# lilinitsy/skele-raytracer

Hardware: AMD Instinct MI355X
Metric: Mrays/sec + frame ms, 1920x1080 gillum=16 spheres2.scn (higher is better)
Workload: dtype f32

## Files before the change

### skele_raytracer_amd/csrc/scene_host.cpp

```cpp
#include "scene_host.h"

#include <cstdarg>
#include <cstdio>
#include <cstdlib>
#include <cstring>
#include <algorithm>
#include <cmath>
#include <fstream>

static thread_local char g_err[512] = "";

void skr_set_error(const char *fmt, ...)
{
	va_list ap;
	va_start(ap, fmt);
	vsnprintf(g_err, sizeof g_err, fmt, ap);
	va_end(ap);
}

extern "C" const char *skr_last_error(void) { return g_err; }

namespace {

int read_floats(const char *p, float *dst, int n)
// ... 218 lines not shown
	const float reach2 = std::nextafter((float) (reach * reach), INFINITY);
	const double D = std::sqrt((double) reach2) * (1.0 + 0x1p-16);
	const double eta = 0x1p-16;
	std::vector<double> cell_dir, cell_theta;
	cube_cells(SKR_SHADOW_CELLS, cell_dir, cell_theta);
	for(double &t : cell_theta) t = t * (1.0 + 0x1p-20) + 0x1p-16;
	std::vector<uint32_t> masks((size_t) nl * SKR_SHADOW_TABLE_WORDS, 0u);
	for(int l = 0; l < nl; l++)
	{
		double lp[3];
		light_pos(l, lp);
		const double lmax = std::max(std::fabs(lp[0]), std::max(std::fabs(lp[1]), std::fabs(lp[2])));
		const double eps_o = 2.0 * std::sqrt(3.0) * (1e-6 + 0x1p-23 * (lmax + D + 1e-6));
		for(int k = 0; k < ns; k++)
		{
			const double q[3] = {sph_geom[k].x - lp[0], sph_geom[k].y - lp[1], sph_geom[k].z - lp[2]};
			const double r2 = sph_geom[k].w, qq = q[0] * q[0] + q[1] * q[1] + q[2] * q[2], qn = std::sqrt(qq);
			const double E = (qn + D + eps_o) * (1.0 + 0x1p-20);
			const double rk = std::sqrt(r2 + 0x1p-16 * (E * E + r2)) + 0x1p-20 * E;
			const double S = qn + rk;
			const double base = rk + eps_o + eta * (S + D + eps_o) / (1.0 - eta) + 0x1p-30 * qn;
			for(int c = 0; c < SKR_SHADOW_TABLE_WORDS; c++)
			{
				const double *wc = &cell_dir[3 * (size_t) c];
				const double s = q[0] * wc[0] + q[1] * wc[1] + q[2] * wc[2];
				const double dist = std::sqrt(std::max(0.0, qq - s * s));
				if(dist <= base + cell_theta[c] * S) masks[(size_t) l * SKR_SHADOW_TABLE_WORDS + c] |= 1u << k;
			}
		}
	}
	shadow_masks.swap(masks);
	shadow_reach2 = reach2;
}

struct BallSphere {
	double v[3], dist;
	double rk;
	double behind, reach;
	bool meets;
};
static BallSphere ball_sphere(const double *q, double rho, const double *C, double r2)
{
	BallSphere b;
	for(int c = 0; c < 3; c++) b.v[c] = C[c] - q[c];
	b.dist = std::sqrt(b.v[0] * b.v[0] + b.v[1] * b.v[1] + b.v[2] * b.v[2]);
	const double E = (b.dist + rho) * (1.0 + 0x1p-20);
	b.rk = std::sqrt(r2 + 0x1p-16 * (E * E + r2)) + 0x1p-20 * E;
	const double tol = 0x1p-30 * (b.dist + rho + b.rk);
	b.behind = rho + 0x1p-16 * E + tol;
	b.reach = b.rk + rho + tol;
	b.meets = b.dist <= b.reach;
	return b;
}
struct ConeSphere {
	double cos_lo, min_sin;
};
static ConeSphere cone_sphere(const double *v, double dist, const double *w, double ct, double st)
{
	const double cp = (v[0] * w[0] + v[1] * w[1] + v[2] * w[2]) / dist;
	const double x = v[1] * w[2] - v[2] * w[1], y = v[2] * w[0] - v[0] * w[2], z = v[0] * w[1] - v[1] * w[0];
	const double sp = std::sqrt(x * x + y * y + z * z) / dist;
	const bool lo0 = cp >= ct;
	const bool hipi = cp <= -ct;
	const double sin_lo = lo0 ? 0.0 : sp * ct - cp * st;
	const double sin_hi = hipi ? 0.0 : sp * ct + cp * st;
	return ConeSphere{lo0 ? 1.0 : cp * ct + sp * st, std::max(0.0, std::min(sin_lo, sin_hi))};
}
static bool cone_ahead(const ConeSphere &c, double dist, double behind) { return dist * c.cos_lo + behind >= 0.0; }
static bool cone_line_touches(const ConeSphere &c, double dist, double reach) { return dist * c.min_sin <= reach; }
static bool ball_cone_touches(const BallSphere &b, const double *w, double ct, double st)
{
	if(b.meets) return true;
	const ConeSphere c = cone_sphere(b.v, b.dist, w, ct, st);
	return cone_ahead(c, b.dist, b.behind) && cone_line_touches(c, b.dist, b.reach);
}
static void gi_ball_bits(const double *q, double rho, const double *C, double r2, uint32_t bit, const std::vector<double> &cell_dir,
						 const std::vector<double> &cth, const std::vector<double> &sth, uint32_t *row)
{
	const BallSphere b = ball_sphere(q, rho, C, r2);
	for(int e = 0; e < SKR_GI_ROW_ENTRIES; e++)
		if(ball_cone_touches(b, &cell_dir[3 * (size_t) e], cth[e], sth[e])) row[e] |= bit;
}

void skr_scene::build_gi_masks()
{
	gi_table.clear();
	gi_grid[0] = gi_grid[1] = SkrGiGrid{};
	gi_mask_word = 0;
	gi_wide = 0;
	const int ns = info.n_spheres;
	if(ns < 1 || ns > SKR_GI_MAX_SPHERES || info.n_triangles > 0) return;
	std::vector<double> C((size_t) 3 * ns), r2(ns), rad(ns);
	for(int k = 0; k < ns; k++)
	{
		C[3 * k] = sph_geom[k].x;
		C[3 * k + 1] = sph_geom[k].y;
		C[3 * k + 2] = sph_geom[k].z;
		r2[k] = sph_geom[k].w;
		rad[k] = std::sqrt(r2[k]);
		for(int c = 0; c < 3; c++)
			if(!(std::fabs(C[3 * k + c]) < 1e6)) return;
		if(!(rad[k] < 1e6)) return;
	}
	std::vector<double> sorted(rad);
	std::sort(sorted.begin(), sorted.end());
	const double small = 4.0 * sorted[ns / 2];
	double flo[3] = {INFINITY, INFINITY, INFINITY}, fhi[3] = {-INFINITY, -INFINITY, -INFINITY}, alo[3] = {INFINITY, INFINITY, INFINITY},
		   ahi[3] = {-INFINITY, -INFINITY, -INFINITY}, rsmall = 0.0;
	for(int k = 0; k < ns; k++)
		for(int c = 0; c < 3; c++)
		{
			alo[c] = std::min(alo[c], C[3 * k + c] - rad[k]);
			ahi[c] = std::max(ahi[c], C[3 * k + c] + rad[k]);
			if(rad[k] <= small)
			{
				flo[c] = std::min(flo[c], C[3 * k + c] - rad[k]);
				fhi[c] = std::max(fhi[c], C[3 * k + c] + rad[k]);
				rsmall = std::max(rsmall, rad[k]);
			}
		}
	double ext_f = 0.0;
	for(int c = 0; c < 3; c++)
	{
		flo[c] -= 2.0 * rsmall;
		fhi[c] += 2.0 * rsmall;
		ext_f = std::max(ext_f, fhi[c] - flo[c]);
	}
	if(!(ext_f > 1e-6)) return;
	double clo[3], chi[3], ext_c = 0.0;
	for(int c = 0; c < 3; c++)
	{
		clo[c] = std::min(flo[c], std::max(alo[c], flo[c] - ext_f));
		chi[c] = std::max(fhi[c], std::min(ahi[c], fhi[c] + ext_f));
		ext_c = std::max(ext_c, chi[c] - clo[c]);
	}
	gi_wide = ns > 16 ? 1 : 0;
	const size_t row_bytes = (size_t) SKR_GI_ROW_ENTRIES * (gi_wide ? 4 : 2);
	struct Cell {
		double q[3], rho;
	};
	std::vector<Cell> cells;
	std::vector<int32_t> index;
	double hh[2] = {0.0, 0.0};
	bool fits = false;
	for(int attempt = 0; attempt < 64 && !fits; attempt++)
	{
		const double grow = std::pow(1.15, attempt);
		cells.clear();
		index.clear();
		for(int g = 0; g < 2; g++)
		{
			SkrGiGrid &G = gi_grid[g];
			const double *lo = g ? clo : flo, *hi = g ? chi : fhi;
			G.inv = (float) (1.0 / ((g ? ext_c / 16.0 : ext_f / 32.0) * grow));
			hh[g] = 1.0 / (double) G.inv;
			for(int c = 0; c < 3; c++)
			{
				float l = (float) lo[c];
				if((double) l > lo[c]) l = std::nextafter(l, -INFINITY);
				G.lo[c] = l;
				G.n[c] = std::max(1, std::min(256, (int) std::ceil((hi[c] - (double) l) / hh[g])));
				G.n_f[c] = (float) G.n[c];
			}
			G.base = (int32_t) index.size();
			const int n0 = G.n[0], n1 = G.n[1], n2 = G.n[2];
			const double pad = 0x1p-18 * std::max(n0, std::max(n1, n2)) * hh[g];
			const double rho = std::sqrt(3.0) * (0.5 * hh[g] + pad) * (1.0 + 0x1p-20);
			for(int k = 0; k < n2; k++)
				for(int j = 0; j < n1; j++)
					for(int i = 0; i < n0; i++)
					{
						const int ijk[3] = {i, j, k};
						Cell cl;
						bool inside_fine = g == 1;
						for(int c = 0; c < 3; c++)
						{
							cl.q[c] = (double) G.lo[c] + (ijk[c] + 0.5) * hh[g];
							const double f0 = (double) gi_grid[0].lo[c], f1 = f0 + gi_grid[0].n[c] * hh[0];
							inside_fine = inside_fine && cl.q[c] - 0.5 * hh[g] >= f0 && cl.q[c] + 0.5 * hh[g] <= f1;
						}
						cl.rho = rho;
						bool near = false;
						for(int s = 0; s < ns && !near && !inside_fine; s++)
						{
							const double dx = C[3 * s] - cl.q[0], dy = C[3 * s + 1] - cl.q[1], dz = C[3 * s + 2] - cl.q[2];
							const double dist = std::sqrt(dx * dx + dy * dy + dz * dz);
							near = std::fabs(dist - rad[s]) <= rho + 1e-4 + 0x1p-16 * (dist + rad[s]);
						}
						index.push_back(near ? (int32_t) cells.size() : -1);
						if(near) cells.push_back(cl);
					}
		}
		fits = ((index.size() + 1) & ~(size_t) 1) * 4 + cells.size() * row_bytes <= SKR_GI_MAX_BYTES;
	}
	if(!fits || cells.empty()) return;
	std::vector<double> cell_dir, cell_theta;
	cube_cells(SKR_GI_DIR_CELLS, cell_dir, cell_theta);
	std::vector<double> cth(SKR_GI_ROW_ENTRIES), sth(SKR_GI_ROW_ENTRIES);
	for(int e = 0; e < SKR_GI_ROW_ENTRIES; e++)
	{
		const double t = cell_theta[e] * (1.0 + 0x1p-20) + 0x1p-40;
		cth[e] = std::cos(t);
		sth[e] = std::sin(t);
	}
	std::vector<uint32_t> masks(cells.size() * SKR_GI_ROW_ENTRIES, 0u);
	for(size_t ci = 0; ci < cells.size(); ci++)
		for(int k = 0; k < ns; k++) gi_ball_bits(cells[ci].q, cells[ci].rho, &C[3 * k], r2[k], 1u << k, cell_dir, cth, sth, &masks[ci * SKR_GI_ROW_ENTRIES]);
	const size_t n_index = (index.size() + 1) & ~(size_t) 1;
	const size_t n_mask_words = gi_wide ? masks.size() : masks.size() / 2;
	std::vector<uint32_t> table((n_index + n_mask_words + 3) & ~(size_t) 3, 0u);
	memcpy(table.data(), index.data(), index.size() * 4);
	if(gi_wide) memcpy(&table[n_index], masks.data(), masks.size() * 4);
	else
		for(size_t e = 0; e < masks.size(); e += 2) table[n_index + e / 2] = masks[e] | masks[e + 1] << 16;
	gi_mask_word = (uint32_t) n_index;
	gi_table.swap(table);
}

struct SurfaceShell {
	float tau;
	double R_lo, R_hi;
};
static SurfaceShell surface_shell(double r2)
{
	SurfaceShell sh;
	sh.tau = std::sqrt(r2) > 1e-3 ? (float) (r2 * 0x1p-7) : -1.0f;
	sh.R_lo = std::sqrt(std::max(0.0, (r2 - sh.tau) * (1.0 - 0x1p-20))) * (1.0 - 0x1p-22);
	sh.R_hi = std::sqrt((r2 + std::max(0.0f, sh.tau)) * (1.0 + 0x1p-20)) * (1.0 + 0x1p-22);
	return sh;
}
static void surface_patch_ball(const double *C, double rad, const SurfaceShell &sh, const double *w, double th, double *q, double &rho)
{
	const double h = rad * std::cos(th);
	for(int c = 0; c < 3; c++) q[c] = C[c] + h * w[c];
	double far = 0.0;
	for(double R : {sh.R_lo, sh.R_hi}) far = std::max(far, std::sqrt(std::max(0.0, R * R + h * h - 2.0 * R * h * std::cos(th))));
	double cmax = 0.0;
	for(int c = 0; c < 3; c++) cmax = std::max(cmax, std::fabs(C[c]));
	rho = far * (1.0 + 0x1p-20) + 0x1p-30 * (cmax + rad);
}
static void surface_cells(int g, std::vector<double> &dir, std::vector<double> &theta)
{
	dir.clear();
	theta.clear();
	if(g) cube_cells(g, dir, theta);
	for(double &t : theta) t = t * (1.0 + 0x1p-20) + 0x1p-20;
}
static double surface_first_edge(const std::vector<double> &rad, const std::vector<double> &r2, double rows)
{
	const int ns = (int) rad.size();
	std::vector<double> sorted(rad);
	std::sort(sorted.begin(), sorted.end());
	double small_area = 0.0;
	for(int k = 0; k < ns; k++)
		if(rad[k] <= 4.0 * sorted[ns / 2]) small_area += 24.0 * r2[k];
	return std::max(1e-6, 0.5 * std::sqrt(small_area / std::max(1.0, rows)));
}

void skr_scene::build_gi_surface()
{
	gi_surface.clear();
	gi_surface_head = 0;
	gi_rows = 0;
	gi_surface_edge = 0.0;
	if(gi_table.empty()) return;
	const int ns = info.n_spheres;
	const size_t row_words = (size_t) SKR_GI_ROW_ENTRIES * (gi_wide ? 4 : 2) / 4;
	gi_rows = (uint32_t) ((gi_table.size() - gi_mask_word) / row_words);
	std::vector<double> C((size_t) 3 * ns), r2(ns), rad(ns), R_lo(ns), R_hi(ns);
	std::vector<float> tau(ns);
	std::vector<SurfaceShell> shell(ns);
	for(int k = 0; k < ns; k++)
	{
		C[3 * k] = sph_geom[k].x;
		C[3 * k + 1] = sph_geom[k].y;
		C[3 * k + 2] = sph_geom[k].z;
		r2[k] = sph_geom[k].w;
		rad[k] = std::sqrt(r2[k]);
		shell[k] = surface_shell(r2[k]);
		tau[k] = shell[k].tau;
		R_lo[k] = shell[k].R_lo;
		R_hi[k] = shell[k].R_hi;
	}
	double blo[3], bhi[3];
	for(int c = 0; c < 3; c++)
	{
		blo[c] = gi_grid[0].lo[c];
		bhi[c] = blo[c] + gi_grid[0].n[c] / (double) gi_grid[0].inv;
	}
	struct Patch {
		int s, cell;
		double q[3], rho;
	};
	std::vector<Patch> patches;
	std::vector<int> G(ns, 0);
	std::vector<std::vector<double>> cdir(ns), cth(ns);
	size_t n_index = 0;
	bool fits = false;
	double edge = surface_first_edge(rad, r2, (double) SKR_GI_MAX_BYTES / (row_words * 4)), used_edge = 0.0;
	for(int attempt = 0; attempt < 200 && !fits; attempt++, edge *= 1.15)
	{
		patches.clear();
		n_index = 0;
		for(int k = 0; k < ns; k++)
		{
			const int g = tau[k] < 0.0f ? 0 : (int) std::min((double) SKR_GI_SURFACE_MAX_CELLS, std::max(1.0, std::ceil(2.0 * rad[k] / edge)));
			if(g != G[k])
			{
				G[k] = g;
				surface_cells(g, cdir[k], cth[k]);
			}
			n_index += (size_t) 6 * g * g;
			for(int cell = 0; cell < 6 * g * g; cell++)
			{
				Patch pt;
				pt.s = k;
				pt.cell = cell;
				surface_patch_ball(&C[3 * k], rad[k], shell[k], &cdir[k][3 * (size_t) cell], cth[k][cell], pt.q, pt.rho);
				double gap2 = 0.0;
				for(int c = 0; c < 3; c++)
				{
					const double o = std::max(0.0, std::max(blo[c] - pt.q[c], pt.q[c] - bhi[c]));
					gap2 += o * o;
				}
				if(gap2 <= pt.rho * pt.rho) patches.push_back(pt);
			}
		}
		fits = (SKR_GI_SURFACE_HEAD * (size_t) ns + n_index) * 4 + patches.size() * row_words * 4 <= SKR_GI_MAX_BYTES;
		if(fits) used_edge = edge;
	}
	if(!fits || patches.empty()) return;
	gi_surface_edge = used_edge;
	std::vector<double> cell_dir, cell_theta;
	cube_cells(SKR_GI_DIR_CELLS, cell_dir, cell_theta);
	std::vector<double> dth(SKR_GI_ROW_ENTRIES), dct(SKR_GI_ROW_ENTRIES), dst(SKR_GI_ROW_ENTRIES);
	for(int e = 0; e < SKR_GI_ROW_ENTRIES; e++)
	{
		dth[e] = cell_theta[e] * (1.0 + 0x1p-20) + 0x1p-40;
		dct[e] = std::cos(dth[e]);
		dst[e] = std::sin(dth[e]);
	}
	std::vector<uint32_t> masks(patches.size() * SKR_GI_ROW_ENTRIES, 0u);
	for(size_t pi = 0; pi < patches.size(); pi++)
	{
		const Patch &pt = patches[pi];
		uint32_t *row = &masks[pi * SKR_GI_ROW_ENTRIES];
		for(int k = 0; k < ns; k++)
			if(k != pt.s) gi_ball_bits(pt.q, pt.rho, &C[3 * k], r2[k], 1u << k, cell_dir, dct, dst, row);
		const int s = pt.s;
		const double *wp = &cdir[s][3 * (size_t) pt.cell];
		const double E = R_hi[s] * (1.0 + 0x1p-20), behind = 0x1p-16 * E + 0x1p-30 * R_hi[s];
		for(int e = 0; e < SKR_GI_ROW_ENTRIES; e++)
		{
			const double *w = &cell_dir[3 * (size_t) e];
			const double x = wp[1] * w[2] - wp[2] * w[1], y = wp[2] * w[0] - wp[0] * w[2], z = wp[0] * w[1] - wp[1] * w[0];
			const double psi = std::atan2(std::sqrt(x * x + y * y + z * z), wp[0] * w[0] + wp[1] * w[1] + wp[2] * w[2]);
			const double ang = psi + cth[s][pt.cell] + dth[e] + 0x1p-30;
			if(!(ang < 0.5 * M_PI && R_lo[s] * std::cos(ang) > behind)) row[e] |= 1u << s;
		}
	}
	const size_t n_mask_words = gi_wide ? masks.size() : masks.size() / 2;
	std::vector<uint32_t> table(n_mask_words + SKR_GI_SURFACE_HEAD * (size_t) ns + n_index, 0u);
	if(gi_wide) memcpy(table.data(), masks.data(), masks.size() * 4);
	else
		for(size_t e = 0; e < masks.size(); e += 2) table[e / 2] = masks[e] | masks[e + 1] << 16;
	uint32_t *head = &table[n_mask_words];
	int32_t *index = reinterpret_cast<int32_t *>(head + SKR_GI_SURFACE_HEAD * ns);
	size_t at = SKR_GI_SURFACE_HEAD * (size_t) ns;
	for(int k = 0; k < ns; k++)
	{
		head[SKR_GI_SURFACE_HEAD * k] = (uint32_t) at;
		head[SKR_GI_SURFACE_HEAD * k + 1] = (uint32_t) G[k];
		const float t = G[k] ? tau[k] : -1.0f;
		memcpy(&head[SKR_GI_SURFACE_HEAD * k + 2], &t, 4);
		for(int c = 0; c < 6 * G[k] * G[k]; c++) head[at + c] = 0xffffffffu;
		at += (size_t) 6 * G[k] * G[k];
	}
	for(size_t pi = 0; pi < patches.size(); pi++)
		index[head[SKR_GI_SURFACE_HEAD * patches[pi].s] - SKR_GI_SURFACE_HEAD * ns + patches[pi].cell] = (int32_t) (gi_rows + pi);
	gi_surface_head = (uint32_t) n_mask_words;
	gi_surface.swap(table);
}

void skr_scene::build_shadow_surface(double rho_scale, double cone_scale)
{
	shadow_surface.clear();
	shadow_surface_head.clear();
	shadow_surface_stride = 0;
	if(shadow_masks.empty()) return;
	const int ns = info.n_spheres, nl = (int) (shadow_masks.size() / SKR_SHADOW_TABLE_WORDS), npairs = (nl + 1) / 2;
	std::vector<double> C((size_t) 3 * ns), r2(ns), rad(ns);
	std::vector<SurfaceShell> shell(ns);
	for(int k = 0; k < ns; k++)
	{
		C[3 * k] = sph_geom[k].x;
		C[3 * k + 1] = sph_geom[k].y;
		C[3 * k + 2] = sph_geom[k].z;
		r2[k] = sph_geom[k].w;
		rad[k] = std::sqrt(r2[k]);
		for(int c = 0; c < 3; c++)
			if(!(std::fabs(C[3 * k + c]) < 1e6)) return;
		if(!(rad[k] < 1e6)) return;
		shell[k] = surface_shell(r2[k]);
	}
	double edge = gi_surface_edge > 0.0 ? gi_surface_edge : surface_first_edge(rad, r2, (double) SKR_GI_MAX_BYTES / (SKR_GI_ROW_ENTRIES * (ns > 16 ? 4 : 2)));
	edge /= SKR_SHADOW_SURFACE_SCALE;
	std::vector<int> G(ns, 0);
	size_t stride = 0;
	for(int attempt = 0; attempt < 200; attempt++, edge *= 1.15)
	{
		stride = 0;
		for(int k = 0; k < ns; k++)
		{
			G[k] = shell[k].tau < 0.0f ? 0 : (int) std::min((double) SKR_GI_SURFACE_MAX_CELLS, std::max(1.0, std::ceil(2.0 * rad[k] / edge)));
			stride += (size_t) 6 * G[k] * G[k];
		}
		if(stride * npairs * 4 <= SKR_SHADOW_SURFACE_MAX_BYTES) break;
	}
	if(stride == 0 || stride * npairs * 4 > SKR_SHADOW_SURFACE_MAX_BYTES) return;
	const uint32_t all = ns >= 32 ? 0xffffffffu : (1u << ns) - 1u;
	const double eta = 0x1p-15;
	std::vector<uint32_t> table(stride * npairs, 0u), head(ns, 0u);
	std::vector<double> cdir, cth;
	std::vector<BallSphere> bs(ns);
	size_t base = 0;
	for(int s = 0; s < ns; s++)
	{
		head[s] = (uint32_t) base | (uint32_t) G[s] << 24;
		surface_cells(G[s], cdir, cth);
		double cmax = 0.0;
		for(int c = 0; c < 3; c++) cmax = std::max(cmax, std::fabs(C[3 * s + c]));
		const double eps_o = 2.0 * std::sqrt(3.0) * (1e-6 + 0x1p-23 * (cmax + shell[s].R_hi + 1e-6));
		const double R_in = shell[s].R_lo - eps_o;
		const double E_own = (shell[s].R_hi + eps_o) * (1.0 + 0x1p-20);
		const double behind_own = 0x1p-16 * E_own + 0x1p-30 * shell[s].R_hi;
		const double tilt = R_in > 0.0 ? std::asin(std::min(1.0, eps_o / shell[s].R_lo)) : 0.0;
		for(int cell = 0; cell < 6 * G[s] * G[s]; cell++)
		{
			const double *wp = &cdir[3 * (size_t) cell];
			double q[3], rho;
			surface_patch_ball(&C[3 * s], rad[s], shell[s], wp, cth[cell], q, rho);
			rho = (rho + eps_o) * rho_scale;
			for(int k = 0; k < ns; k++)
				if(k != s) bs[k] = ball_sphere(q, rho, &C[3 * k], r2[k]);
			for(int l = 0; l < nl; l++)
			{
				uint32_t &word = table[(size_t) (l >> 1) * stride + base + cell];
				const skr_f4 &lp = lights[2 * (size_t) l];
				const double d[3] = {lp.x - q[0], lp.y - q[1], lp.z - q[2]};
				const double dl = std::sqrt(d[0] * d[0] + d[1] * d[1] + d[2] * d[2]);
				if(!(dl > rho * (1.0 + 0x1p-20) + 0x1p-30 * (cmax + rad[s])))
				{
					word = all;
					continue;
				}
				const double w[3] = {d[0] / dl, d[1] / dl, d[2] / dl};
				const double theta = (std::asin(std::min(1.0, rho / dl)) * (1.0 + 0x1p-20) + eta) * cone_scale;
				const double ct = std::cos(theta), st = std::sin(theta);
				const double near_l = eps_o + eta * (dl + rho) * (1.0 + 0x1p-20);
				const double lpd[3] = {lp.x, lp.y, lp.z};
				for(int k = 0; k < ns; k++)
				{
					if(k == s) continue;
					const BallSphere &b = bs[k];
					const bool ahead = b.meets || cone_ahead(cone_sphere(b.v, b.dist, w, ct, st), b.dist, b.behind);
					const double vl[3] = {C[3 * k] - lpd[0], C[3 * k + 1] - lpd[1], C[3 * k + 2] - lpd[2]};
					const double distl = std::sqrt(vl[0] * vl[0] + vl[1] * vl[1] + vl[2] * vl[2]);
					const double reach_l = b.rk + near_l + 0x1p-30 * (distl + dl + b.rk);
					const bool line = distl <= reach_l || cone_line_touches(cone_sphere(vl, distl, w, ct, st), distl, reach_l);
					if(ahead && line) word |= 1u << k;
				}
				const double x = wp[1] * w[2] - wp[2] * w[1], y = wp[2] * w[0] - wp[0] * w[2], z = wp[0] * w[1] - wp[1] * w[0];
				const double psi = std::atan2(std::sqrt(x * x + y * y + z * z), wp[0] * w[0] + wp[1] * w[1] + wp[2] * w[2]);
				const double ang = psi + cth[cell] + tilt + theta + 0x1p-30;
				if(!(R_in > 0.0 && ang < 0.5 * M_PI && R_in * std::cos(ang) > behind_own)) word |= 1u << s;
			}
		}
		base += (size_t) 6 * G[s] * G[s];
	}
	shadow_surface_stride = (uint32_t) stride;
	shadow_surface.swap(table);
	shadow_surface_head.swap(head);
}

void skr_scene::build_triangle_chunks()
{
	tri_chunks.clear();
	tri_any_cone = false;
// ... 981 lines not shown
}

static int get_culling_set(const skr_scene *scene, const std::vector<skr_f4> &sets, int32_t level, int32_t *chunk_size, int32_t *n_nodes, int32_t *n_chunks,
						   float *device_tris, float *node_spheres, int32_t *node_links, float *chunk_spheres)
{
	if(!scene || level < 0 || level >= SKR_CULL_LEVELS) return SKR_ERR_ARG;
	const int nt = scene->info.n_triangles, nn = nt ? scene->tri_node_count : 0, cs = scene->tri_chunk_size;
	const int nc = nt ? (nt + cs - 1) / cs : 0;
	if(chunk_size) *chunk_size = cs;
	if(n_nodes) *n_nodes = nn;
	if(n_chunks) *n_chunks = nc;
	if(device_tris && nt) memcpy(device_tris, scene->tris.data(), (size_t) nt * 48);
	const skr_f4 *base = sets.data() + (size_t) level * scene->tri_chunk_stride;
	for(int i = 0; i < nn; i++)
	{
		if(node_spheres) memcpy(node_spheres + 8 * (size_t) i, base + 3 * (size_t) i, 32);
		if(node_links) memcpy(node_links + 4 * (size_t) i, base + 3 * (size_t) i + 2, 16);
	}
	if(chunk_spheres && nc) memcpy(chunk_spheres, base + 3 * ((size_t) nn + 1), (size_t) nc * 32);
	return SKR_OK;
}

int skr_scene_get_culling(const skr_scene *scene, int32_t level, int32_t *chunk_size, int32_t *n_nodes, int32_t *n_chunks,
						  float *device_tris, float *node_spheres, int32_t *node_links, float *chunk_spheres)
{
	return get_culling_set(scene, scene ? scene->tri_chunks : std::vector<skr_f4>(), level, chunk_size, n_nodes, n_chunks, device_tris, node_spheres, node_links, chunk_spheres);
}

int skr_scene_get_trace_culling(const skr_scene *scene, int32_t level, int32_t *chunk_size, int32_t *n_nodes, int32_t *n_chunks,
								float *device_tris, float *node_spheres, int32_t *node_links, float *chunk_spheres, float ball[4])
{
	if(scene && ball) memcpy(ball, scene->trace_ball, 16);
	return get_culling_set(scene, scene ? scene->trace_chunks : std::vector<skr_f4>(), level, chunk_size, n_nodes, n_chunks, device_tris, node_spheres, node_links, chunk_spheres);
}

int skr_scene_get_shadow_masks(const skr_scene *scene, int32_t *n_lights, int32_t *cells, float *reach2, uint32_t *masks)
{
	if(!scene) return SKR_ERR_ARG;
	if(n_lights) *n_lights = (int32_t) (scene->shadow_masks.size() / SKR_SHADOW_TABLE_WORDS);
	if(cells) *cells = SKR_SHADOW_CELLS;
	if(reach2) *reach2 = scene->shadow_reach2;
	if(masks && !scene->shadow_masks.empty()) memcpy(masks, scene->shadow_masks.data(), scene->shadow_masks.size() * 4);
	return SKR_OK;
}

int skr_scene_get_gi_masks(const skr_scene *scene, int32_t *n_words, int32_t *mask_word, int32_t *wide, int32_t *dir_cells, float *grids, uint32_t *table)
{
	if(!scene) return SKR_ERR_ARG;
	if(n_words) *n_words = (int32_t) scene->gi_table.size();
	if(mask_word) *mask_word = (int32_t) scene->gi_mask_word;
	if(wide) *wide = scene->gi_wide;
	if(dir_cells) *dir_cells = SKR_GI_DIR_CELLS;
	if(grids)
		for(int g = 0; g < 2; g++)
		{
			const SkrGiGrid &G = scene->gi_grid[g];
			const float row[8] = {G.lo[0], G.lo[1], G.lo[2], G.inv, (float) G.n[0], (float) G.n[1], (float) G.n[2], (float) G.base};
			memcpy(grids + 8 * g, row, sizeof(row));
		}
	if(table && !scene->gi_table.empty()) memcpy(table, scene->gi_table.data(), scene->gi_table.size() * 4);
	return SKR_OK;
}

int skr_scene_get_gi_surface(const skr_scene *scene, int32_t *n_words, int32_t *head_word, int32_t *first_row, uint32_t *table)
{
	if(!scene) return SKR_ERR_ARG;
	if(n_words) *n_words = (int32_t) scene->gi_surface.size();
	if(head_word) *head_word = (int32_t) scene->gi_surface_head;
	if(first_row) *first_row = (int32_t) scene->gi_rows;
	if(table && !scene->gi_surface.empty()) memcpy(table, scene->gi_surface.data(), scene->gi_surface.size() * 4);
	return SKR_OK;
}

int skr_scene_get_shadow_surface(const skr_scene *scene, int32_t *n_pairs, int32_t *stride, uint32_t *head, uint32_t *table)
{
	if(!scene) return SKR_ERR_ARG;
	if(stride) *stride = (int32_t) scene->shadow_surface_stride;
	if(n_pairs) *n_pairs = scene->shadow_surface_stride ? (int32_t) (scene->shadow_surface.size() / scene->shadow_surface_stride) : 0;
	if(head && !scene->shadow_surface_head.empty()) memcpy(head, scene->shadow_surface_head.data(), scene->shadow_surface_head.size() * 4);
	if(table && !scene->shadow_surface.empty()) memcpy(table, scene->shadow_surface.data(), scene->shadow_surface.size() * 4);
	return SKR_OK;
}

int skr_scene_rebuild_shadow_surface(skr_scene *scene, double rho_scale, double cone_scale)
{
	if(!scene) return SKR_ERR_ARG;
	scene->build_shadow_surface(rho_scale, cone_scale);
	return SKR_OK;
}

void skr_options_default(skr_options *opt)
{
	if(!opt) return;
	opt->width = 1920;
	opt->height = 1080;
	opt->fov = 60;
	opt->monte_carlo = 0;
	opt->num_path_traces = 1;
	opt->grid_size = 0;
	opt->max_depth = 3;
	opt->use_shadows = 0;
	opt->seed = 1;
	opt->shade_triangles = 0;
	opt->progressive_passes = 1;
	opt->legacy_reflect = 0;
}

uint64_t skr_radiance_ray_count(const skr_options *opt)
{
	if(!opt || opt->width <= 0 || opt->height <= 0) return 0;
	const uint64_t S = opt->grid_size > 0 ? (uint64_t) opt->grid_size * opt->grid_size : 1;
	uint64_t per = 0, pw = 1;
	for(int k = 0; k < opt->max_depth; k++)
	{
		per += pw;
		if(!opt->monte_carlo) break;
		pw *= (uint64_t) (opt->num_path_traces > 0 ? opt->num_path_traces : 0);
	}
	const uint64_t K = opt->progressive_passes > 1 ? (uint64_t) opt->progressive_passes : 1;
	return (uint64_t) opt->width * opt->height * S * per * K;
}

int skr_write_ppm(const char *path, uint32_t width, uint32_t height, const uint8_t *rgb)
{
	if(!path || !rgb) return SKR_ERR_ARG;
	std::ofstream ofs(path, std::ios::out | std::ios::binary);
	if(!ofs)
	{
		skr_set_error("cannot open '%s' for writing", path);
		return SKR_ERR_IO;
	}
	ofs << "P6\n" << width << " " << height << "\n255\n";
	ofs.write(reinterpret_cast<const char *>(rgb), (std::streamsize) width * height * 3);
	ofs.close();
	return ofs ? SKR_OK : SKR_ERR_IO;
}


int skr_write_pfm(const char *path, uint32_t width, uint32_t height, const float *rgbf)
{
	if(!path || !rgbf) return SKR_ERR_ARG;
	std::ofstream ofs(path, std::ios::out | std::ios::binary);
	if(!ofs)
	{
		skr_set_error("cannot open '%s' for writing", path);
		return SKR_ERR_IO;
	}
	ofs << "PF\n" << width << " " << height << "\n-1.0\n";
	for(uint32_t y = height; y-- > 0;) ofs.write(reinterpret_cast<const char *>(rgbf + (size_t) y * width * 3), (std::streamsize) width * 12);
	ofs.close();
	return ofs ? SKR_OK : SKR_ERR_IO;
}

int skr_write_png(const char *path, uint32_t width, uint32_t height, const uint8_t *rgb)
{
	if(!path || !rgb || width == 0 || height == 0) return SKR_ERR_ARG;
	static uint32_t crc_table[256];
	static bool have_table = false;
	if(!have_table)
	{
		for(uint32_t n = 0; n < 256; n++)
		{
			uint32_t c = n;
			for(int k = 0; k < 8; k++) c = (c & 1u) ? 0xedb88320u ^ (c >> 1) : c >> 1;
			crc_table[n] = c;
		}
// ... 66 lines not shown
```

### skele_raytracer_amd/csrc/scene_host.h

```cpp
#pragma once

#include <cstdint>
#include <string>
#include <vector>

#include "../../include/skr.h"
#include "shadow_cells.h"
#include "tri_chunks.h"


struct skr_f4 {
	float x, y, z, w;
};

struct skr_scene {
	std::vector<float> raw_spheres;
	std::vector<float> raw_sphere_ior;
	std::vector<float> raw_triangles;
	std::vector<float> raw_triangle_materials;
	std::vector<float> raw_point_lights;
	std::vector<float> raw_directional_lights;
	std::vector<float> raw_fog;
	std::vector<float> raw_spot_lights;
	std::vector<float> light_radii;
	bool strict = false;
	bool triangle_shadows = false;
	bool sphere_tree = false;
	skr_scene_info info{};

	std::vector<skr_f4> sph_geom;
	std::vector<skr_f4> sph_amb;
	std::vector<skr_f4> sph_kd;
	std::vector<skr_f4> sph_ks;
	std::vector<skr_f4> lights;
	std::vector<skr_f4> spot_cones;
	std::vector<skr_f4> tris;
	std::vector<skr_f4> tri_mats;
	std::vector<skr_f4> tri_chunks;
	int tri_chunk_size = SKR_TRI_CHUNK_MIXED;

	void finalize();
	void build_lights();
	int n_spot() const { return (int) (raw_spot_lights.size() / 11); }
	bool soft() const
	{
		for(float r : light_radii)
			if(r > 0.0f) return true;
		return false;
	}
	size_t tri_chunk_stride = 0;
	int tri_node_count = 0;
	bool tri_any_cone = false;
	void build_triangle_chunks();
	std::vector<int> tri_order;
	void build_triangle_materials();
	void build_triangle_chunk_level(double d_max, std::vector<skr_f4> &out, const double *origin_ball = nullptr);
	std::vector<skr_f4> trace_chunks;
	float trace_ball[4] = {0.0f, 0.0f, 0.0f, 0.0f};
	bool trace_any_cone = false;
	std::vector<uint32_t> shadow_masks;
	float shadow_reach2 = 0.0f;
	void build_shadow_masks();
	std::vector<uint32_t> gi_table;
	SkrGiGrid gi_grid[2] = {};
	uint32_t gi_mask_word = 0;
	int gi_wide = 0;
	void build_gi_masks();
	std::vector<uint32_t> gi_surface;
	uint32_t gi_surface_head = 0;
	uint32_t gi_rows = 0;
	double gi_surface_edge = 0.0;
	void build_gi_surface();
	std::vector<uint32_t> shadow_surface, shadow_surface_head;
	uint32_t shadow_surface_stride = 0;
	void build_shadow_surface(double rho_scale = 1.0, double cone_scale = 1.0);
};

#define SKR_SPHERE_CHUNK 4
#define SKR_SPHERE_SUPER 8
struct SkrSphereTree {
	int n_nodes = 0, n_chunks = 0, n_always = 0;
	std::vector<skr_f4> rows;
	std::vector<int32_t> file;
	std::vector<skr_f4> nodes;
	std::vector<skr_f4> chunks;
	float ball[4] = {0.0f, 0.0f, 0.0f, -1.0f};
};
void skr_build_sphere_tree(const skr_scene &scene, SkrSphereTree &out);

bool skr_spot_row_ok(const float row[11]);

int skr_parse_scn(const std::string &path, bool echo, uint32_t flags, skr_scene &out);

void skr_set_error(const char *fmt, ...);
```

### skele_raytracer_amd/csrc/shadow_cells.h

```cpp
#pragma once

#include <stdint.h>

#ifndef SKR_SHADOW_CELLS
#define SKR_SHADOW_CELLS 32
#endif
#define SKR_SHADOW_TABLE_WORDS (6 * SKR_SHADOW_CELLS * SKR_SHADOW_CELLS)
#define SKR_SHADOW_MAX_SPHERES 32

#define SKR_SURFACE_SLACK 0x1p-7f
#ifndef SKR_SHADOW_SURFACE_SCALE
#define SKR_SHADOW_SURFACE_SCALE 4
#endif
#define SKR_SHADOW_SURFACE_MAX_BYTES (1u << 20)

#ifndef SKR_GI_DIR_CELLS
#define SKR_GI_DIR_CELLS 16
#endif
#define SKR_GI_ROW_ENTRIES (6 * SKR_GI_DIR_CELLS * SKR_GI_DIR_CELLS)
#define SKR_GI_MAX_SPHERES 32
#define SKR_GI_MAX_BYTES (2u << 20)
struct SkrGiGrid {
	float lo[3], inv;
	float n_f[3];
	int32_t n[3], base;
};

#define SKR_GI_SURFACE_HEAD 4
#define SKR_GI_SURFACE_MAX_CELLS 128
```

Baseline: 64290.

## Rebalance GI occlusion mask budgets and add far surface patches with coarser directions

Halves the GI direction-cell resolution (16 to 8 per cube face) and splits the mask memory budget into grid, near-surface and far-surface pools. Surface patches outside the fine grid box are now kept, sorted by distance, with optionally scaled radii and cones, and big spheres get coarser patch edges. The shadow surface edge is derived from a separate reference layout rather than the GI edge. The aim is to make GI rays more likely to resolve occluder candidates from small precomputed tables, at the cost of coarser direction cones that may let more spheres through each lookup.

New measurement: 64280 (median of 2 runs). Within noise of the previous version (-0.0%).

```diff
diff --git a/skele_raytracer_amd/csrc/scene_host.cpp b/skele_raytracer_amd/csrc/scene_host.cpp
--- a/skele_raytracer_amd/csrc/scene_host.cpp
+++ b/skele_raytracer_amd/csrc/scene_host.cpp
@@ -324,51 +324,53 @@
 		if(ball_cone_touches(b, &cell_dir[3 * (size_t) e], cth[e], sth[e])) row[e] |= bit;
 }
 
-void skr_scene::build_gi_masks()
-{
-	gi_table.clear();
-	gi_grid[0] = gi_grid[1] = SkrGiGrid{};
-	gi_mask_word = 0;
-	gi_wide = 0;
-	const int ns = info.n_spheres;
-	if(ns < 1 || ns > SKR_GI_MAX_SPHERES || info.n_triangles > 0) return;
-	std::vector<double> C((size_t) 3 * ns), r2(ns), rad(ns);
-	for(int k = 0; k < ns; k++)
-	{
-		C[3 * k] = sph_geom[k].x;
-		C[3 * k + 1] = sph_geom[k].y;
-		C[3 * k + 2] = sph_geom[k].z;
-		r2[k] = sph_geom[k].w;
-		rad[k] = std::sqrt(r2[k]);
-		for(int c = 0; c < 3; c++)
-			if(!(std::fabs(C[3 * k + c]) < 1e6)) return;
-		if(!(rad[k] < 1e6)) return;
-	}
+static double small_sphere_box(const std::vector<double> &C, const std::vector<double> &rad, double *flo, double *fhi)
+{
+	const int ns = (int) rad.size();
 	std::vector<double> sorted(rad);
 	std::sort(sorted.begin(), sorted.end());
 	const double small = 4.0 * sorted[ns / 2];
-	double flo[3] = {INFINITY, INFINITY, INFINITY}, fhi[3] = {-INFINITY, -INFINITY, -INFINITY}, alo[3] = {INFINITY, INFINITY, INFINITY},
-		   ahi[3] = {-INFINITY, -INFINITY, -INFINITY}, rsmall = 0.0;
+	double rsmall = 0.0;
+	for(int c = 0; c < 3; c++)
+	{
+		flo[c] = INFINITY;
+		fhi[c] = -INFINITY;
+	}
 	for(int k = 0; k < ns; k++)
 		for(int c = 0; c < 3; c++)
-		{
-			alo[c] = std::min(alo[c], C[3 * k + c] - rad[k]);
-			ahi[c] = std::max(ahi[c], C[3 * k + c] + rad[k]);
 			if(rad[k] <= small)
 			{
 				flo[c] = std::min(flo[c], C[3 * k + c] - rad[k]);
 				fhi[c] = std::max(fhi[c], C[3 * k + c] + rad[k]);
 				rsmall = std::max(rsmall, rad[k]);
 			}
-		}
-	double ext_f = 0.0;
+	double ext = 0.0;
 	for(int c = 0; c < 3; c++)
 	{
 		flo[c] -= 2.0 * rsmall;
 		fhi[c] += 2.0 * rsmall;
-		ext_f = std::max(ext_f, fhi[c] - flo[c]);
-	}
-	if(!(ext_f > 1e-6)) return;
+		ext = std::max(ext, fhi[c] - flo[c]);
+	}
+	return ext;
+}
+
+struct GiGridCell {
+	double q[3], rho;
+};
+static bool gi_grid_layout(const std::vector<double> &C, const std::vector<double> &rad, size_t bytes, size_t row_bytes, SkrGiGrid *grid,
+						   std::vector<GiGridCell> &cells, std::vector<int32_t> &index)
+{
+	typedef GiGridCell Cell;
+	const int ns = (int) rad.size();
+	double flo[3], fhi[3], alo[3] = {INFINITY, INFINITY, INFINITY}, ahi[3] = {-INFINITY, -INFINITY, -INFINITY};
+	for(int k = 0; k < ns; k++)
+		for(int c = 0; c < 3; c++)
+		{
+			alo[c] = std::min(alo[c], C[3 * k + c] - rad[k]);
+			ahi[c] = std::max(ahi[c], C[3 * k + c] + rad[k]);
+		}
+	const double ext_f = small_sphere_box(C, rad, flo, fhi);
+	if(!(ext_f > 1e-6)) return false;
 	double clo[3], chi[3], ext_c = 0.0;
 	for(int c = 0; c < 3; c++)
 	{
@@ -376,13 +378,6 @@
 		chi[c] = std::max(fhi[c], std::min(ahi[c], fhi[c] + ext_f));
 		ext_c = std::max(ext_c, chi[c] - clo[c]);
 	}
-	gi_wide = ns > 16 ? 1 : 0;
-	const size_t row_bytes = (size_t) SKR_GI_ROW_ENTRIES * (gi_wide ? 4 : 2);
-	struct Cell {
-		double q[3], rho;
-	};
-	std::vector<Cell> cells;
-	std::vector<int32_t> index;
 	double hh[2] = {0.0, 0.0};
 	bool fits = false;
 	for(int attempt = 0; attempt < 64 && !fits; attempt++)
@@ -392,7 +387,7 @@
 		index.clear();
 		for(int g = 0; g < 2; g++)
 		{
-			SkrGiGrid &G = gi_grid[g];
+			SkrGiGrid &G = grid[g];
 			const double *lo = g ? clo : flo, *hi = g ? chi : fhi;
 			G.inv = (float) (1.0 / ((g ? ext_c / 16.0 : ext_f / 32.0) * grow));
 			hh[g] = 1.0 / (double) G.inv;
@@ -418,7 +413,7 @@
 						for(int c = 0; c < 3; c++)
 						{
 							cl.q[c] = (double) G.lo[c] + (ijk[c] + 0.5) * hh[g];
-							const double f0 = (double) gi_grid[0].lo[c], f1 = f0 + gi_grid[0].n[c] * hh[0];
+							const double f0 = (double) grid[0].lo[c], f1 = f0 + grid[0].n[c] * hh[0];
 							inside_fine = inside_fine && cl.q[c] - 0.5 * hh[g] >= f0 && cl.q[c] + 0.5 * hh[g] <= f1;
 						}
 						cl.rho = rho;
@@ -433,9 +428,41 @@
 						if(near) cells.push_back(cl);
 					}
 		}
-		fits = ((index.size() + 1) & ~(size_t) 1) * 4 + cells.size() * row_bytes <= SKR_GI_MAX_BYTES;
-	}
-	if(!fits || cells.empty()) return;
+		fits = ((index.size() + 1) & ~(size_t) 1) * 4 + cells.size() * row_bytes <= bytes;
+	}
+	return fits && !cells.empty();
+}
+
+void skr_scene::build_gi_masks()
+{
+	gi_table.clear();
+	gi_grid[0] = gi_grid[1] = SkrGiGrid{};
+	gi_mask_word = 0;
+	gi_wide = 0;
+	const int ns = info.n_spheres;
+	if(ns < 1 || ns > SKR_GI_MAX_SPHERES || info.n_triangles > 0) return;
+	std::vector<double> C((size_t) 3 * ns), r2(ns), rad(ns);
+	for(int k = 0; k < ns; k++)
+	{
+		C[3 * k] = sph_geom[k].x;
+		C[3 * k + 1] = sph_geom[k].y;
+		C[3 * k + 2] = sph_geom[k].z;
+		r2[k] = sph_geom[k].w;
+		rad[k] = std::sqrt(r2[k]);
+		for(int c = 0; c < 3; c++)
+			if(!(std::fabs(C[3 * k + c]) < 1e6)) return;
+		if(!(rad[k] < 1e6)) return;
+	}
+	gi_wide = ns > 16 ? 1 : 0;
+	const size_t row_bytes = (size_t) SKR_GI_ROW_ENTRIES * (gi_wide ? 4 : 2);
+	std::vector<GiGridCell> cells;
+	std::vector<int32_t> index;
+	if(!gi_grid_layout(C, rad, SKR_GI_GRID_BYTES, row_bytes, gi_grid, cells, index))
+	{
+		gi_grid[0] = gi_grid[1] = SkrGiGrid{};
+		gi_wide = 0;
+		return;
+	}
 	std::vector<double> cell_dir, cell_theta;
 	cube_cells(SKR_GI_DIR_CELLS, cell_dir, cell_theta);
 	std::vector<double> cth(SKR_GI_ROW_ENTRIES), sth(SKR_GI_ROW_ENTRIES);
@@ -499,7 +526,77 @@
 	return std::max(1e-6, 0.5 * std::sqrt(small_area / std::max(1.0, rows)));
 }
 
-void skr_scene::build_gi_surface()
+struct SurfacePatch {
+	int s, cell;
+	double q[3], rho, gap;
+};
+struct SurfaceLayout {
+	std::vector<int> G;
+	std::vector<std::vector<double>> cdir, cth;
+	std::vector<SurfacePatch> near, far;
+	size_t n_index = 0;
+};
+static void surface_layout(double edge, const std::vector<double> &C, const std::vector<double> &rad, const std::vector<SurfaceShell> &shell,
+						   const double *blo, const double *bhi, double big_scale, bool want_far, SurfaceLayout &L)
+{
+	const int ns = (int) rad.size();
+	std::vector<double> sorted(rad);
+	std::sort(sorted.begin(), sorted.end());
+	const double small = 4.0 * sorted[ns / 2];
+	L.G.resize(ns, 0);
+	L.cdir.resize(ns);
+	L.cth.resize(ns);
+	L.near.clear();
+	L.far.clear();
+	L.n_index = 0;
+	for(int k = 0; k < ns; k++)
+	{
+		const double ek = rad[k] <= small ? edge : edge * big_scale;
+		const int g = shell[k].tau < 0.0f ? 0 : (int) std::min((double) SKR_GI_SURFACE_MAX_CELLS, std::max(1.0, std::ceil(2.0 * rad[k] / ek)));
+		if(g != L.G[k] || (g && L.cth[k].empty()))
+		{
+			L.G[k] = g;
+			surface_cells(g, L.cdir[k], L.cth[k]);
+		}
+		L.n_index += (size_t) 6 * g * g;
+		for(int cell = 0; cell < 6 * g * g; cell++)
+		{
+			SurfacePatch pt;
+			pt.s = k;
+			pt.cell = cell;
+			surface_patch_ball(&C[3 * k], rad[k], shell[k], &L.cdir[k][3 * (size_t) cell], L.cth[k][cell], pt.q, pt.rho);
+			double gap2 = 0.0;
+			for(int c = 0; c < 3; c++)
+			{
+				const double o = std::max(0.0, std::max(blo[c] - pt.q[c], pt.q[c] - bhi[c]));
+				gap2 += o * o;
+			}
+			pt.gap = 0.0;
+			if(gap2 > pt.rho * pt.rho)
+			{
+				double d2 = 0.0;
+				for(int c = 0; c < 3; c++) d2 += (pt.q[c] - 0.5 * (blo[c] + bhi[c])) * (pt.q[c] - 0.5 * (blo[c] + bhi[c]));
+				pt.gap = std::max(std::sqrt(d2), 1e-300);
+			}
+			if(pt.gap == 0.0) L.near.push_back(pt);
+			else if(want_far) L.far.push_back(pt);
+		}
+	}
+}
+static double surface_fit_edge(size_t bytes, size_t row_bytes, const std::vector<double> &C, const std::vector<double> &rad, const std::vector<double> &r2,
+							   const std::vector<SurfaceShell> &shell, const double *blo, const double *bhi, double big_scale, bool want_far, SurfaceLayout &L)
+{
+	const size_t ns = rad.size();
+	double edge = surface_first_edge(rad, r2, (double) bytes / row_bytes);
+	for(int attempt = 0; attempt < 200; attempt++, edge *= 1.15)
+	{
+		surface_layout(edge, C, rad, shell, blo, bhi, big_scale, want_far, L);
+		if((SKR_GI_SURFACE_HEAD * ns + L.n_index) * 4 + L.near.size() * row_bytes <= bytes) return L.near.empty() ? 0.0 : edge;
+	}
+	return 0.0;
+}
+
+void skr_scene::build_gi_surface(double far_rho_scale, double far_theta_scale)
 {
 	gi_surface.clear();
 	gi_surface_head = 0;
@@ -530,48 +627,20 @@
 		blo[c] = gi_grid[0].lo[c];
 		bhi[c] = blo[c] + gi_grid[0].n[c] / (double) gi_grid[0].inv;
 	}
-	struct Patch {
-		int s, cell;
-		double q[3], rho;
-	};
-	std::vector<Patch> patches;
-	std::vector<int> G(ns, 0);
-	std::vector<std::vector<double>> cdir(ns), cth(ns);
-	size_t n_index = 0;
-	bool fits = false;
-	double edge = surface_first_edge(rad, r2, (double) SKR_GI_MAX_BYTES / (row_words * 4)), used_edge = 0.0;
-	for(int attempt = 0; attempt < 200 && !fits; attempt++, edge *= 1.15)
-	{
-		patches.clear();
-		n_index = 0;
-		for(int k = 0; k < ns; k++)
-		{
-			const int g = tau[k] < 0.0f ? 0 : (int) std::min((double) SKR_GI_SURFACE_MAX_CELLS, std::max(1.0, std::ceil(2.0 * rad[k] / edge)));
-			if(g != G[k])
-			{
-				G[k] = g;
-				surface_cells(g, cdir[k], cth[k]);
-			}
-			n_index += (size_t) 6 * g * g;
-			for(int cell = 0; cell < 6 * g * g; cell++)
-			{
-				Patch pt;
-				pt.s = k;
-				pt.cell = cell;
-				surface_patch_ball(&C[3 * k], rad[k], shell[k], &cdir[k][3 * (size_t) cell], cth[k][cell], pt.q, pt.rho);
-				double gap2 = 0.0;
-				for(int c = 0; c < 3; c++)
-				{
-					const double o = std::max(0.0, std::max(blo[c] - pt.q[c], pt.q[c] - bhi[c]));
-					gap2 += o * o;
-				}
-				if(gap2 <= pt.rho * pt.rho) patches.push_back(pt);
-			}
-		}
-		fits = (SKR_GI_SURFACE_HEAD * (size_t) ns + n_index) * 4 + patches.size() * row_words * 4 <= SKR_GI_MAX_BYTES;
-		if(fits) used_edge = edge;
-	}
-	if(!fits || patches.empty()) return;
+	SurfaceLayout L;
+	const double used_edge = surface_fit_edge(SKR_GI_NEAR_BYTES, row_words * 4, C, rad, r2, shell, blo, bhi, SKR_GI_SURFACE_BIG_SCALE, true, L);
+	if(!(used_edge > 0.0)) return;
+	const size_t near_bytes = (SKR_GI_SURFACE_HEAD * (size_t) ns + L.n_index) * 4 + L.near.size() * row_words * 4;
+	const size_t far_rows = std::min(L.far.size(), ((size_t) SKR_GI_NEAR_BYTES + SKR_GI_FAR_BYTES - near_bytes) / (row_words * 4));
+	std::stable_sort(L.far.begin(), L.far.end(), [](const SurfacePatch &a, const SurfacePatch &b) { return a.gap < b.gap; });
+	L.far.resize(far_rows);
+	const size_t n_near = L.near.size();
+	std::vector<SurfacePatch> &patches = L.near;
+	patches.insert(patches.end(), L.far.begin(), L.far.end());
+	for(size_t pi = n_near; pi < patches.size(); pi++) patches[pi].rho *= far_rho_scale;
+	const std::vector<int> &G = L.G;
+	const std::vector<std::vector<double>> &cdir = L.cdir, &cth = L.cth;
+	const size_t n_index = L.n_index;
 	gi_surface_edge = used_edge;
 	std::vector<double> cell_dir, cell_theta;
 	cube_cells(SKR_GI_DIR_CELLS, cell_dir, cell_theta);
@@ -585,7 +654,7 @@
 	std::vector<uint32_t> masks(patches.size() * SKR_GI_ROW_ENTRIES, 0u);
 	for(size_t pi = 0; pi < patches.size(); pi++)
 	{
-		const Patch &pt = patches[pi];
+		const SurfacePatch &pt = patches[pi];
 		uint32_t *row = &masks[pi * SKR_GI_ROW_ENTRIES];
 		for(int k = 0; k < ns; k++)
 			if(k != pt.s) gi_ball_bits(pt.q, pt.rho, &C[3 * k], r2[k], 1u << k, cell_dir, dct, dst, row);
@@ -597,7 +666,7 @@
 			const double *w = &cell_dir[3 * (size_t) e];
 			const double x = wp[1] * w[2] - wp[2] * w[1], y = wp[2] * w[0] - wp[0] * w[2], z = wp[0] * w[1] - wp[1] * w[0];
 			const double psi = std::atan2(std::sqrt(x * x + y * y + z * z), wp[0] * w[0] + wp[1] * w[1] + wp[2] * w[2]);
-			const double ang = psi + cth[s][pt.cell] + dth[e] + 0x1p-30;
+			const double ang = psi + cth[s][pt.cell] * (pi < n_near ? 1.0 : far_theta_scale) + dth[e] + 0x1p-30;
 			if(!(ang < 0.5 * M_PI && R_lo[s] * std::cos(ang) > behind)) row[e] |= 1u << s;
 		}
 	}
@@ -645,7 +714,26 @@
 		if(!(rad[k] < 1e6)) return;
 		shell[k] = surface_shell(r2[k]);
 	}
-	double edge = gi_surface_edge > 0.0 ? gi_surface_edge : surface_first_edge(rad, r2, (double) SKR_GI_MAX_BYTES / (SKR_GI_ROW_ENTRIES * (ns > 16 ? 4 : 2)));
+	const size_t ref_row = (size_t) 6 * SKR_SHADOW_SURFACE_REF_CELLS * SKR_SHADOW_SURFACE_REF_CELLS * (ns > 16 ? 4 : 2);
+	double edge = 0.0;
+	if(ns <= SKR_GI_MAX_SPHERES && info.n_triangles == 0)
+	{
+		SkrGiGrid grid[2] = {};
+		std::vector<GiGridCell> cells;
+		std::vector<int32_t> index;
+		if(gi_grid_layout(C, rad, SKR_SHADOW_SURFACE_REF_BYTES, ref_row, grid, cells, index))
+		{
+			double blo[3], bhi[3];
+			for(int c = 0; c < 3; c++)
+			{
+				blo[c] = grid[0].lo[c];
+				bhi[c] = blo[c] + grid[0].n[c] / (double) grid[0].inv;
+			}
+			SurfaceLayout L;
+			edge = surface_fit_edge(SKR_SHADOW_SURFACE_REF_BYTES, ref_row, C, rad, r2, shell, blo, bhi, 1.0, false, L);
+		}
+	}
+	if(!(edge > 0.0)) edge = surface_first_edge(rad, r2, (double) SKR_SHADOW_SURFACE_REF_BYTES / ref_row);
 	edge /= SKR_SHADOW_SURFACE_SCALE;
 	std::vector<int> G(ns, 0);
 	size_t stride = 0;
@@ -1793,6 +1881,13 @@
 	return SKR_OK;
 }
 
+int skr_scene_rebuild_gi_surface(skr_scene *scene, double far_rho_scale, double far_theta_scale)
+{
+	if(!scene) return SKR_ERR_ARG;
+	scene->build_gi_surface(far_rho_scale, far_theta_scale);
+	return SKR_OK;
+}
+
 int skr_scene_rebuild_shadow_surface(skr_scene *scene, double rho_scale, double cone_scale)
 {
 	if(!scene) return SKR_ERR_ARG;
diff --git a/skele_raytracer_amd/csrc/scene_host.h b/skele_raytracer_amd/csrc/scene_host.h
--- a/skele_raytracer_amd/csrc/scene_host.h
+++ b/skele_raytracer_amd/csrc/scene_host.h
@@ -70,7 +70,7 @@
 	uint32_t gi_surface_head = 0;
 	uint32_t gi_rows = 0;
 	double gi_surface_edge = 0.0;
-	void build_gi_surface();
+	void build_gi_surface(double far_rho_scale = 1.0, double far_theta_scale = 1.0);
 	std::vector<uint32_t> shadow_surface, shadow_surface_head;
 	uint32_t shadow_surface_stride = 0;
 	void build_shadow_surface(double rho_scale = 1.0, double cone_scale = 1.0);
diff --git a/skele_raytracer_amd/csrc/shadow_cells.h b/skele_raytracer_amd/csrc/shadow_cells.h
--- a/skele_raytracer_amd/csrc/shadow_cells.h
+++ b/skele_raytracer_amd/csrc/shadow_cells.h
@@ -12,14 +12,25 @@
 #ifndef SKR_SHADOW_SURFACE_SCALE
 #define SKR_SHADOW_SURFACE_SCALE 4
 #endif
+#define SKR_SHADOW_SURFACE_REF_CELLS 16
+#define SKR_SHADOW_SURFACE_REF_BYTES (2u << 20)
 #define SKR_SHADOW_SURFACE_MAX_BYTES (1u << 20)
 
 #ifndef SKR_GI_DIR_CELLS
-#define SKR_GI_DIR_CELLS 16
+#define SKR_GI_DIR_CELLS 8
 #endif
 #define SKR_GI_ROW_ENTRIES (6 * SKR_GI_DIR_CELLS * SKR_GI_DIR_CELLS)
 #define SKR_GI_MAX_SPHERES 32
-#define SKR_GI_MAX_BYTES (2u << 20)
+#ifndef SKR_GI_BUDGET_BYTES
+#define SKR_GI_BUDGET_BYTES (5u << 19)
+#endif
+#ifndef SKR_GI_GRID_BYTES
+#define SKR_GI_GRID_BYTES (1u << 19)
+#endif
+#ifndef SKR_GI_NEAR_BYTES
+#define SKR_GI_NEAR_BYTES (5u << 18)
+#endif
+#define SKR_GI_FAR_BYTES (SKR_GI_BUDGET_BYTES - SKR_GI_GRID_BYTES - SKR_GI_NEAR_BYTES)
 struct SkrGiGrid {
 	float lo[3], inv;
 	float n_f[3];
@@ -27,4 +38,7 @@
 };
 
 #define SKR_GI_SURFACE_HEAD 4
+#ifndef SKR_GI_SURFACE_BIG_SCALE
+#define SKR_GI_SURFACE_BIG_SCALE 2.5
+#endif
 #define SKR_GI_SURFACE_MAX_CELLS 128
```
